# zhuker/lamejs

Measured on NVIDIA H100. Metric: encoded audio seconds/sec (44.1kHz stereo 128kbps CBR), higher is better.
Workload: dtype f64

## Files before the change

lamejs_b200/csrc/k_quant.cuh:

```cuda
#ifndef MP3B200_K_QUANT_CUH
#define MP3B200_K_QUANT_CUH
#include <stddef.h>
#include "mp3_device.cuh"
#include "mp3_tables.h"
#include "k_psy.cuh"

#define Q_LARGE_BITS 100000
#define Q_IXMAX 8206
#define Q_FULL 0xffffffffu

struct GranuleInfoDev {
  int global_gain, part2_3_length, part2_length, big_values, count1, scalefac_compress;
  int table_select[3], region0_count, region1_count, preflag, scalefac_scale, count1table_select, block_type;
  int subblock_gain[4];
  int count1bits, sfbmax, sfbdivide, sfb_lmax, psymax, psy_lmax, sfb_smin, max_nonzero_coeff;
  int scalefac[MP3_SFBMAX];
  int slen[4];
  int part_row;
  int pad_;
  double xrpow_max;
};
struct QuantFrameState {
  int stream, rel_frame;
  int in_old[2], in_step[2];
// ... 9 lines not shown
#define Q_R1S(ch) (4 << (ch))
#define Q_R1(ch) (16 << (ch))
#define Q_R0_ANY 3
#define Q_R1_ANY 48
#define Q_R1S_ANY 12
struct GcPrep { float xmin[MP3_SFBMAX]; int have, mnz, block_type; double xrpow_max; };

__device__ unsigned short g_huff_code[1666];
__device__ unsigned char g_huff_len[1666];
__constant__ int c_huff_off[34];
__constant__ int c_huff_xlen[34];
__device__ int g_t32l[16];
__device__ int g_t33l[16];
__constant__ int c_slen1_n[16];
__constant__ int c_slen2_n[16];
__device__ int g_slen_n[2][16];
__device__ int g_scale_tab[2][16];
__device__ unsigned int g_cat_tab[8][256];
__constant__ int c_slen1_tab[16];
__constant__ int c_slen2_tab[16];
__constant__ int c_huf_noesc[15];

static int quant_upload_constants() {
  static const int t32l[16] = {1, 5, 5, 7, 5, 8, 7, 9, 5, 7, 7, 9, 7, 9, 9, 10};
  static const int t33l[16] = {4, 5, 5, 6, 5, 6, 6, 7, 5, 6, 6, 7, 6, 7, 7, 8};
  static const int s1n[16] = {1, 1, 1, 1, 8, 2, 2, 2, 4, 4, 4, 8, 8, 8, 16, 16};
  static const int s2n[16] = {1, 2, 4, 8, 1, 2, 4, 8, 2, 4, 8, 2, 4, 8, 4, 8};
  static const int s1t[16] = {0, 0, 0, 0, 3, 1, 1, 1, 2, 2, 2, 3, 3, 3, 4, 4};
  static const int s2t[16] = {0, 1, 2, 3, 0, 1, 2, 3, 1, 2, 3, 1, 2, 3, 2, 3};
  static const int ss[16] = {0, 18, 36, 54, 54, 36, 54, 72, 54, 72, 90, 72, 90, 108, 108, 126};
// ... 16 lines not shown
        unsigned a = 0, b = 0, d = 0;
        if (x < xl && y < xl) {
          const int i = x * xl + y;
          if (c == 0) a = b = d = MP3_HUFF_LEN[MP3_HUFF_OFF[1] + i];
          else if (c == 1) { a = MP3_HUFF_TABLE23[i] >> 16; b = d = MP3_HUFF_TABLE23[i] & 0xffff; }
          else if (c == 2) { a = MP3_HUFF_TABLE56[i] >> 16; b = d = MP3_HUFF_TABLE56[i] & 0xffff; }
          else { a = MP3_HUFF_LEN[MP3_HUFF_OFF[t1] + i]; b = MP3_HUFF_LEN[MP3_HUFF_OFF[t1 + 1] + i]; d = MP3_HUFF_LEN[MP3_HUFF_OFF[t1 + 2] + i]; }
        }
        ct[c][q] = a | (b << 11) | (d << 22);
      }
      { const unsigned a = MP3_HUFF_LARGETBL[q] >> 16, b = MP3_HUFF_LARGETBL[q] & 0xffff; ct[6][q] = a | (b << 11) | (b << 22); }
      ct[7][q] = 0;
    }
    UP(g_slen_n, sn); UP(g_scale_tab, st); UP(g_cat_tab, ct);
  }
#undef UP
  return 0;
}

struct __align__(16) GcWork {
  float xrpow[576];
  short ixw[576];
  short* ixg;
  GranuleInfoDev w, b;
  const Mp3Geo* geo;
  float xmin[MP3_SFBMAX], distort[MP3_SFBMAX];
  int pn_step[MP3_SFBMAX]; float pn_noise[MP3_SFBMAX], pn_noise_log[MP3_SFBMAX];
  int pn_global_gain, pn_sfb_count1;
  unsigned char mode[MP3_SFBMAX + 1];
  short nstart[MP3_SFBMAX], nlen[MP3_SFBMAX];
// ... 4 lines not shown
struct __align__(16) WarpShared {
  double ath[6];
  int scfsi[4];
  GcWork wk;
};
#define Q_STRIDE_NOXR ((int)((offsetof(WarpShared, wk) + offsetof(GcWork, xr) + 15) & ~(size_t)15))
static_assert((offsetof(WarpShared, wk) + offsetof(GcWork, xr)) % 16 == 0 && (offsetof(WarpShared, wk) + offsetof(GcWork, xrpow)) % 16 == 0 &&
              (offsetof(WarpShared, wk) + offsetof(GcWork, ixw)) % 16 == 0 && sizeof(WarpShared) % 16 == 0, "rows are moved as 16-byte vectors");
#ifndef Q_SLIM_BLOCKS
#define Q_SLIM_BLOCKS 9
#endif

#define LANE (threadIdx.x & 31)
#ifdef Q_TASKSTAT
__device__ int g_taskstat[1 << 16][8];
#endif
#ifdef Q_STATS
__device__ unsigned long long g_qstats[16];
#define QSTAT(i) do { if (LANE == 0) atomicAdd(&g_qstats[i], 1ull); } while (0)
#else
#define QSTAT(i) do { } while (0)
#endif
#define Q_PRAGMA(x) _Pragma(#x)
#define Q_UNROLL(n) Q_PRAGMA(unroll n)
#ifndef Q_RT_UNROLL
#define Q_RT_UNROLL 1
#endif
#ifndef Q_CB_UNROLL
#define Q_CB_UNROLL 1
#endif
// ... 82 lines not shown
#ifdef MP3_DOMAIN_CHECK
  {
    unsigned fa = 0, fb = 0, fc = 0;
    for (int p = p0; p < p1; p += 32) {
      const unsigned v = rc.cat == 6 ? pair_bits(w32[p], 6, rc.lin) : __ldg(&g_cat_tab[rc.cat][((w32[p] & 0xfu) << 4) | (w32[p] >> 16)]);
      fa += v & 0x7ffu; fb += (v >> 11) & 0x7ffu; fc += v >> 22;
    }
    DOMAIN_MISS(DOM_BITSUM_FIELD, fa > 0x7ffu || fb > 0x7ffu || fc > 0x3ffu || wsumu(fa) > 0xffffu || wsumu(fb) > 0xffffu);
  }
#endif
  const unsigned ab = wsumu((s & 0x7ffu) | (((s >> 11) & 0x7ffu) << 16));
  const int c = wsum((int)(s >> 22));
  return region_pick(mx, rc, (int)(ab & 0xffffu), (int)(ab >> 16), c, bits);
}

__device__ __forceinline__ int noquant_count_bits_w(const Mp3Tables* T, const short* ix, GranuleInfoDev* gi, GcWork* wk, bool use_prev, int top) {
  const int lane = LANE;
  const unsigned* w32 = reinterpret_cast<const unsigned*>(ix);
  const int count1 = wmax(top);
  int a1 = 0, a2 = 0, nq = 0;
  const int qmax = count1 >> 2;
  bool stop = false;
#pragma unroll 1
  for (int q0 = 0; q0 < qmax && !stop; q0 += 32) {
    const int q = q0 + lane;
    int bad = 1, v1 = 0, v2 = 0;
    if (q < qmax) {
      const int i = count1 - 4 * q;
      const unsigned wa = w32[(i - 4) >> 1], wb = w32[(i - 2) >> 1];
      if (((wa | wb) & 0xfffefffeu) == 0) {
        bad = 0;
        const int p = (int)(((wa & 1u) << 3) | ((wa >> 16) << 2) | ((wb & 1u) << 1) | (wb >> 16));
        v1 = __ldg(&g_t32l[p]); v2 = __ldg(&g_t33l[p]);
      }
    }
    const unsigned m = __ballot_sync(Q_FULL, bad);
    const int first_bad = m ? __ffs(m) - 1 : 32;
    if (lane >= first_bad) { v1 = 0; v2 = 0; }
    a1 += wsum(v1); a2 += wsum(v2);
    nq += first_bad;
    if (first_bad < 32) stop = true;
  }
  if (nq > qmax) nq = qmax;
  const int bigv = count1 - 4 * nq;
  int bits = a1, c1sel = 0;
  if (a1 > a2) { bits = a2; c1sel = 1; }
  const int count1bits = bits;
  int r0 = gi->region0_count, r1 = gi->region1_count;
  int ts0 = gi->table_select[0], ts1 = gi->table_select[1], ts2 = gi->table_select[2];
  if (bigv != 0) {
    int b1, b2;
    const int bt = gi->block_type;
    if (bt == BT_SHORT) {
      b1 = 3 * T->sfb_s[3];
      b2 = bigv;
    } else if (bt == BT_NORM) {
      b1 = r0 = T->bv_scf[bigv - 2];
      b2 = r1 = T->bv_scf[bigv - 1];
      b2 = T->sfb_l[b1 + b2 + 2];
      b1 = T->sfb_l[b1 + 1];
    } else {
      r0 = 7; r1 = 22 - 1 - 7 - 1;
      b1 = T->sfb_l[7 + 1];
      b2 = bigv;
    }
    b1 = min(b1, bigv);
    b2 = min(b2, bigv);
    if (bt == BT_NORM && b2 < bigv) { QSTAT(15); ts2 = region_table_w(ix, b2, bigv, &bits); }
    if (0 < b1) { QSTAT(15); ts0 = region_table_w(ix, 0, b1, &bits); }
    if (b1 < b2) { QSTAT(15); ts1 = region_table_w(ix, b1, b2, &bits); }
  }
  __syncwarp();
  if (lane == 0) {
    gi->count1 = count1; gi->count1table_select = c1sel; gi->count1bits = count1bits; gi->big_values = bigv;
    gi->region0_count = r0; gi->region1_count = r1;
    gi->table_select[0] = ts0; gi->table_select[1] = ts1; gi->table_select[2] = ts2;
    if (use_prev) {
      int sc = 0;
      if (bigv != 0 && gi->block_type == BT_NORM) {
        if (bigv >= 576) sc = 22;
        else { sc = T->geo[0].sfb_of_line[bigv]; if (T->sfb_l[sc] != bigv) sc++; }
      }
      wk->pn_sfb_count1 = sc;
    }
  }
  __syncwarp();
  return bits;
}

__device__ __forceinline__ int pretab_of(int sfb) { return sfb < 22 ? (int)((0x2fe95400000ull >> (2 * sfb)) & 3ull) : 0; }

__device__ __forceinline__ int sfb_step(const GranuleInfoDev* gi, const GcWork* wk, int sfb) {
  return gi->global_gain - ((gi->scalefac[sfb] + (gi->preflag != 0 ? pretab_of(sfb) : 0)) << (gi->scalefac_scale + 1)) -
         gi->subblock_gain[wk->geo->window[sfb]] * 8;
}

template <bool use_prev>
__device__ __forceinline__ int count_bits_w(const Mp3Tables* T, GcWork* wk, GranuleInfoDev* gi, short* ix) {
  const int lane = LANE;
  const double istep = (double)T->ipow20[gi->global_gain];
  if (gi->xrpow_max > T->ixmax_over_istep[gi->global_gain]) return Q_LARGE_BITS;
  const int sfbmax = gi->block_type == BT_SHORT ? 38 : 21;
  const int mnz = gi->max_nonzero_coeff;
  unsigned* iw32 = reinterpret_cast<unsigned*>(ix);
  const int i0h = min(576, ((mnz + 2) >> 1) << 1) >> 1;
  if (!use_prev) {
    const int qend = (mnz + 1) & ~1;
    int top = 0;
Q_UNROLL(Q_CB_UNROLL)
    for (int p = lane; p < 288; p += 32) {
      unsigned v = 0;
      if (2 * p < qend) {
        const float2 xp = *reinterpret_cast<const float2*>(&wk->xrpow[2 * p]);
        double x0 = (double)xp.x * istep, x1 = (double)xp.y * istep;
        x0 += (double)__ldg(&T->adj43[js_trunc<DOM_TRUNC_QUANT>(x0)]);
        x1 += (double)__ldg(&T->adj43[js_trunc<DOM_TRUNC_QUANT>(x1)]);
// ... 23 lines not shown
      }
      wk->mode[sfb] = (unsigned char)md;
      wk->nstart[sfb] = jst;
    }
    const unsigned m = __ballot_sync(Q_FULL, trunc_here);
    if (m && term == sfbmax + 1) term = s0 + __ffs(m) - 1;
  }
  __syncwarp();
  int zero_from = 576;
  if (term <= sfbmax) {
    const int term_len = mnz - wk->nstart[term] + 1;
    zero_from = term_len > 0 ? ((term_len & 1) ? mnz : mnz + 1) : mnz;
    if (lane == 0) wk->mode[term] = 1;
  }
  __syncwarp();
  const double compare01 = T->cmp01_over_istep[gi->global_gain];
  int top = 0;
Q_UNROLL(Q_CB_UNROLL)
  for (int p = lane; p < 288; p += 32) {
    const int i = 2 * p;
    unsigned v;
    if (i >= zero_from) { v = 0; iw32[p] = 0; }
    else {
      const int md = wk->mode[wk->geo->sfb_of_line[i]];
      const bool z1 = (i + 1) >= zero_from;
      if (md == 0) {
        v = iw32[p];
        if (z1) { v &= 0xffffu; iw32[p] = v; }
      } else {
        const float2 xp = *reinterpret_cast<const float2*>(&wk->xrpow[i]);
        unsigned v0, v1;
        if (md == 2) { v0 = (compare01 > (double)xp.x) ? 0u : 1u; v1 = (compare01 > (double)xp.y) ? 0u : 1u; }
        else {
          double x0 = (double)xp.x * istep, x1 = (double)xp.y * istep;
          x0 += (double)__ldg(&T->adj43[js_trunc<DOM_TRUNC_QUANT>(x0)]);
          x1 += (double)__ldg(&T->adj43[js_trunc<DOM_TRUNC_QUANT>(x1)]);
          v0 = (unsigned)js_trunc<DOM_TRUNC_QUANT>(x0); v1 = (unsigned)js_trunc<DOM_TRUNC_QUANT>(x1);
          DOMAIN_MISS(DOM_PACK_OUTER, x0 >= 32768.0 || x1 >= 32768.0);
        }
        if (z1) v1 = 0;
        v = v0 | (v1 << 16);
        iw32[p] = v;
      }
    }
    if (v != 0 && p < i0h) top = 2 * p + 2;
  }
  __syncwarp();
  return noquant_count_bits_w(T, ix, gi, wk, use_prev, top);
}

struct NoiseRes { int over_count; double over_SSD, max_noise; int bits; };
__device__ __forceinline__ void calc_noise_w(const Mp3Tables* T, GcWork* wk, const GranuleInfoDev* gi, const short* ix, NoiseRes* res) {
  const int lane = LANE;
  const int psymax = gi->psymax, mnz = gi->max_nonzero_coeff;
  int first_trunc = psymax;
#pragma unroll 1
  for (int s0 = 0; s0 < psymax; s0 += 32) {
    const int sfb = s0 + lane;
    int crosses = 0;
    if (sfb < psymax) {
      const int j = wk->geo->start[sfb], w = wk->geo->width[sfb];
      if (wk->pn_step[sfb] == sfb_step(gi, wk, sfb)) wk->nlen[sfb] = -1;
      else { wk->nstart[sfb] = (short)j; wk->nlen[sfb] = (short)(w >> 1); crosses = (j + w) > mnz; }
    }
    const unsigned m = __ballot_sync(Q_FULL, crosses);
    if (m && first_trunc == psymax) first_trunc = s0 + __ffs(m) - 1;
  }
  __syncwarp();
  if (lane == 0 && first_trunc < psymax) {
    int j = wk->geo->start[first_trunc];
#pragma unroll 1
    for (int sfb = first_trunc; sfb < psymax; sfb++) {
      const int w = wk->geo->width[sfb];
      if (wk->nlen[sfb] < 0) { j += w; continue; }
      int l = w >> 1;
      if ((j + w) > mnz) { const int us = mnz - j + 1; l = us > 0 ? us >> 1 : 0; }
      wk->nstart[sfb] = (short)j; wk->nlen[sfb] = (short)l;
      j += 2 * l;
    }
  }
  __syncwarp();
  int over = 0, ssd = 0; double mxn = -20.0;
#pragma unroll 1
  for (int s0 = 0; s0 < psymax; s0 += 32) {
    const int sfb = s0 + lane;
    if (sfb < psymax) {
      const int s = sfb_step(gi, wk, sfb);
      const bool cached = wk->nlen[sfb] < 0;
      double noise;
      if (cached) noise = (double)wk->pn_noise[sfb];
      else {
        const double step = (double)T->pow20[s + MP3_QMAX2];
        int j = wk->nstart[sfb];
        noise = 0;
Q_UNROLL(Q_CN_UNROLL)
        for (int l = wk->nlen[sfb]; l > 0; l--, j += 2) {
          const float2 x = *reinterpret_cast<const float2*>(&wk->xr[j]);
          const unsigned q0 = reinterpret_cast<const unsigned short*>(ix)[j], q1 = reinterpret_cast<const unsigned short*>(ix)[j + 1];
          double temp;
          temp = fabs((double)x.x) - (double)__ldg(&T->pow43[q0]) * step; noise += temp * temp;
          temp = fabs((double)x.y) - (double)__ldg(&T->pow43[q1]) * step; noise += temp * temp;
        }
        wk->pn_step[sfb] = s;
        { f32s t; t = noise; wk->pn_noise[sfb] = t.v; }
      }
      noise = noise / (double)wk->xmin[sfb];
      { f32s t; t = noise; wk->distort[sfb] = t.v; }
      if (cached) noise = (double)wk->pn_noise_log[sfb];
      else {
        noise = q_log10(js_dmax(noise, 1E-20));
        { f32s t; t = noise; wk->pn_noise_log[sfb] = t.v; }
      }
      if (noise > 0.0) {
        int tmp = js_trunc<DOM_TRUNC_NOISE>(noise * 10 + .5);
        if (tmp < 1) tmp = 1;
        ssd += tmp * tmp;
        over++;
      }
      mxn = js_dmax(mxn, noise);
    }
  }
#pragma unroll 1
  for (int o = 16; o > 0; o >>= 1) {
    const double other = __shfl_xor_sync(Q_FULL, mxn, o);
    mxn = js_dmax(mxn, other);
  }
  over = wsum(over);
  if (lane == 0) wk->pn_global_gain = gi->global_gain;
  __syncwarp();
  res->over_count = over; res->over_SSD = (double)wsum(ssd); res->max_noise = mxn;
}

__device__ __forceinline__ bool scale_bitcount_w(GranuleInfoDev* gi) {
  const int lane = LANE;
  int* scalefac = gi->scalefac;
  const bool is_short = gi->block_type == BT_SHORT;
  const int sfbmax = gi->sfbmax, sfbdivide = gi->sfbdivide;
  __syncwarp();
  if (!is_short && 0 == gi->preflag) {
    const bool in = lane >= 11 && lane < 21;
    const int pt = pretab_of(lane);
    const bool ok = !in || scalefac[lane] >= pt;
    if (__all_sync(Q_FULL, ok)) {
      __syncwarp();
      if (in) scalefac[lane] -= pt;
// ... 45 lines not shown
  return mode_gr == 2 ? scale_bitcount_w(gi) : scale_bitcount_lsf_w(gi);
}

__device__ __forceinline__ bool loop_break_w(const GranuleInfoDev* gi, const GcWork* wk) {
  bool nz = true;
#pragma unroll 1
  for (int sfb = LANE; sfb < gi->sfbmax; sfb += 32)
    if (gi->scalefac[sfb] + gi->subblock_gain[wk->geo->window[sfb]] == 0) nz = false;
  return __all_sync(Q_FULL, nz);
}

__device__ __forceinline__ void scale_xrpow_w(GcWork* wk, GranuleInfoDev* gi, double f34) {
  const int lane = LANE;
  const int sfbmax = gi->sfbmax;
  float mx = 0.0f;
#pragma unroll 1
  for (int p = lane; p < 288; p += 32) {
    const int sfb = wk->geo->sfb_of_line[2 * p];
    if (sfb < sfbmax && wk->mode[sfb]) {
      float2* xp = reinterpret_cast<float2*>(&wk->xrpow[2 * p]);
      float2 x = *xp;
      f32s v0, v1; v0.v = x.x; v1.v = x.y;
      v0 *= f34; v1 *= f34;
      x.x = v0.v; x.y = v1.v;
      *xp = x;
      mx = fmaxf(mx, fmaxf(v0.v, v1.v));
    }
  }
#pragma unroll 1
  for (int o = 16; o > 0; o >>= 1) mx = fmaxf(mx, __shfl_xor_sync(Q_FULL, mx, o));
  if (lane == 0 && (double)mx > gi->xrpow_max) gi->xrpow_max = (double)mx;
  __syncwarp();
}
// ... 89 lines not shown
    const int sfbmax = gi->sfbmax;
    double trigger = 0;
#pragma unroll 1
    for (int sfb = lane; sfb < sfbmax; sfb += 32) if (trigger < (double)wk->distort[sfb]) trigger = (double)wk->distort[sfb];
    for (int o = 16; o > 0; o >>= 1) { const double t = __shfl_xor_sync(Q_FULL, trigger, o); if (trigger < t) trigger = t; }
    if (trigger > 1.0) trigger = sqrt(trigger);
    else trigger *= .95;
#pragma unroll 1
    for (int sfb = lane; sfb < sfbmax; sfb += 32) {
      const int amp = !((double)wk->distort[sfb] < trigger);
      wk->mode[sfb] = (unsigned char)amp;
      if (amp) gi->scalefac[sfb]++;
    }
  }
  __syncwarp();
  scale_xrpow_w(wk, gi, ifq);
  int r;
  if (loop_break_w(gi, wk)) r = 0;
  else r = scale_bitcount_any_w(gi, T->mode_gr) ? 2 : 1;
  if (r == 0) return false;
  if (r == 1) return true;
  return balance_escalate_w(T, wk);
}

__device__ __forceinline__ void copy_gi_w(GranuleInfoDev* dst, const GranuleInfoDev* src) {
  const int n = sizeof(GranuleInfoDev) / 4;
  const int* s = reinterpret_cast<const int*>(src);
  int* d = reinterpret_cast<int*>(dst);
  __syncwarp();
  static_assert(sizeof(GranuleInfoDev) / 4 <= 96, "three rounds");
  int v[3];
#pragma unroll
  for (int k = 0; k < 3; k++) { const int i = LANE + 32 * k; if (i < n) v[k] = s[i]; }
#pragma unroll
  for (int k = 0; k < 3; k++) { const int i = LANE + 32 * k; if (i < n) d[i] = v[k]; }
  __syncwarp();
}
// ... 54 lines not shown

__device__ __forceinline__ unsigned long long gi_hash(const GranuleInfoDev* gi) {
  const unsigned* w = reinterpret_cast<const unsigned*>(gi);
  unsigned sum = 0, x = 0;
#pragma unroll 1
  for (int i = LANE; i < (int)(sizeof(GranuleInfoDev) / 4); i += 32) {
    unsigned v = (w[i] ^ ((unsigned)i * 0x9E3779B9u)) * 0x85EBCA6Bu;
    v ^= v >> 13; v *= 0xC2B2AE35u; v ^= v >> 16;
    sum += v; x ^= __funnelshift_l(v, v, i & 31);
  }
  sum = __reduce_add_sync(Q_FULL, sum);
  x = __reduce_xor_sync(Q_FULL, x);
  return ((unsigned long long)sum << 32) | x;
}

__device__ __forceinline__ void outer_loop_w(const Mp3Tables* T, GcWork* wk, int targ_bits) {
  const int lane = LANE;
  NoiseRes best, cur;
  int best_part2_3_length = 9999999;
#pragma unroll 1
  for (int i = lane; i < MP3_SFBMAX; i += 32) { wk->pn_step[i] = 0; wk->pn_noise[i] = 0.0f; wk->pn_noise_log[i] = 0.0f; }
  if (lane == 0) { wk->pn_global_gain = 0; wk->pn_sfb_count1 = 0; }
  __syncwarp();
  calc_noise_w(T, wk, &wk->b, wk->ixw, &best);
  best.bits = wk->b.part2_3_length;
  copy_gi_w(&wk->w, &wk->b);
  bool best_here = true;
  int age = 0;
  const int quant_comp = T->quant_comp;
  (void)quant_comp;
  do {
    const int search_limit = 3;
    int maxggain = 255;
    if (!balance_noise_w(T, wk)) break;
    GranuleInfoDev* w = &wk->w;
    if (w->scalefac_scale != 0) maxggain = 254;
    const int huff_bits = targ_bits - w->part2_length;
    if (huff_bits <= 0) break;
    int p23, gg;
    if (best_here) { copy_ix_w(wk->ixg, wk->ixw); best_here = false; }
    int sc_in;
    for (;;) {
      sc_in = wk->pn_sfb_count1;
      QSTAT(8);
      p23 = count_bits_w<true>(T, wk, w, wk->ixw);
      gg = w->global_gain;
      __syncwarp();
      if (!(p23 > huff_bits && gg <= maxggain)) break;
      if (lane == 0) w->global_gain = gg + 1;
      __syncwarp();
    }
    if (lane == 0) w->part2_3_length = p23;
    __syncwarp();
    if (gg > maxggain) break;
    if (best.over_count == 0) {
      bool repeat = wk->pn_sfb_count1 == sc_in;
      for (;;) {
        if (!repeat) { QSTAT(9); p23 = count_bits_w<true>(T, wk, w, wk->ixw); }
        repeat = false;
        gg = w->global_gain;
        __syncwarp();
        if (!(p23 > best_part2_3_length && gg <= maxggain)) break;
        if (lane == 0) w->global_gain = gg + 1;
        __syncwarp();
      }
      if (lane == 0) w->part2_3_length = p23;
      __syncwarp();
      if (gg > maxggain) break;
    }
    QSTAT(10);
    calc_noise_w(T, wk, w, wk->ixw, &cur);
    cur.bits = w->part2_3_length;
    bool better;
    if (best.over_count > 0) {
      better = cur.over_SSD <= best.over_SSD;
      if (cur.over_SSD == best.over_SSD) better = cur.bits < best.bits;
    } else {
      better = ((cur.max_noise < 0) && ((cur.max_noise * 10 + cur.bits) <= (best.max_noise * 10 + best.bits)));
    }
    if (best.over_count == 0) better = better && cur.bits < best.bits;
    if (better) {
      best_part2_3_length = wk->b.part2_3_length;
      best = cur;
      copy_gi_w(&wk->b, &wk->w);
      best_here = true;
      age = 0;
    } else {
      if (++age > search_limit && best.over_count == 0) break;
    }
    const int cont = (wk->w.global_gain + wk->w.scalefac_scale) < 255;
    __syncwarp();
    if (!cont) break;
  } while (true);
  if (!best_here) copy_ix_w(wk->ixw, wk->ixg);
}

__device__ __noinline__ double ath_adjust_dev(double a, double x, double athFloor) {
  const double o = 90.30873362, p = 94.82444863;
  double u = q_log10(x) * 10.0;
  const double v = a * a;
  double w = 0.0;
  u -= athFloor;
  if (v > 1E-20) w = 1. + q_log10(v) * (10.0 / o);
  if (w < 0) w = 0.;
  u *= w;
  u += athFloor + o - p;
  return q_pow(10., 0.1 * u);
}

// ... 655 lines not shown
  if (t > 4095) t = 4095;
  int targ = (int)t;
  const int bits = targ * nch;
  if (bits > 7680) { targ = targ * 7680; targ = (int)((double)targ / bits); }
  (void)ch;
  return targ;
}

#ifndef Q_WARPS
#define Q_WARPS 4
#endif
#ifndef Q_BLOCKS_PER_SM
#define Q_BLOCKS_PER_SM 7
#endif
#define Q_THREADS (32 * Q_WARPS)

__device__ __forceinline__ int next_task(int* counter) {
  int t = 0;
  if (LANE == 0) t = atomicAdd(counter, 1);
  return __shfl_sync(Q_FULL, t, 0);
}
template <int STRIDE = (int)sizeof(WarpShared)>
__device__ __forceinline__ WarpShared* warp_shared() {
  extern __shared__ __align__(16) unsigned char smem_raw[];
  return reinterpret_cast<WarpShared*>(smem_raw + (threadIdx.x >> 5) * STRIDE);
}
__device__ __forceinline__ void gi_init_w(GranuleInfoDev* gi, const GcPrep* __restrict__ pr) {
  __syncwarp();
  int* w = reinterpret_cast<int*>(gi);
#pragma unroll 1
// ... 84 lines not shown
  for (int t = next_task(counter); t < ntasks; t = next_task(counter)) {
    const int wi = t / nch, ch = t - wi * nch;
    const int frow = list ? list[wi] : wi;
    QuantFrameState* q = qs + frow;
    const int flags = revalidate ? q->redo : 0;
    if (revalidate == 3 && (flags & Q_R0_ANY)) continue;
    if (revalidate && gr == 1 && !(flags & (Q_R0_ANY | Q_R1S(ch)))) continue;
    const FrameGeom fg = frame_geom(T, streams, q);
    const StreamDesc& sd = streams[fg.z];
    const size_t urow = (size_t)sd.unit_base + T->mode_gr * fg.f + gr, gidx = urow * nch + ch;
    const int targ = granule_budget(nch, fg.mean_bits, gr, q->used0[0], q->used0[1], ch);
    int ov = gr == 0 ? q->in_old[ch] : q->bs_gain0[ch];
    int cs = gr == 0 ? q->in_step[ch] : q->bs_step0[ch];
    const GcPrep* pr = prep + gidx;
    const bool have = pr->have != 0;
    gi_init_w(&wk->b, pr);
    if (lane == 0) wk->geo = &T->geo[pr->block_type == BT_SHORT ? 1 : 0];
    unsigned long long h = 0;
    if (have) {
      copy_row16_w(wk->xrpow, xrpow_g + gidx * 576, 2304);
      QSTAT(revalidate ? 12 + gr : 11);
      bin_search_w(T, wk, targ, &ov, &cs, revalidate ? 2 + 2 * gr : 0);
      h = gi_hash(&wk->b);
    } else {
      __syncwarp();
#pragma unroll 1
      for (int i = lane; i < 288; i += 32) reinterpret_cast<unsigned*>(wk->ixw)[i] = 0;
      __syncwarp();
    }
    bool store;
// ... 25 lines not shown
        q->out_step[ch] = cs;
        if (store) { q->out_old[ch] = ov; q->bs_hash[1][ch] = h; atomicOr(&q->redo, Q_R1(ch)); }
      }
    }
    if (store) {
      copy_row16_w(l3enc + gidx * 576, wk->ixw, 1152);
      copy_gi_w(&ginfo[gidx], &wk->b);
    }
  }
}

__global__ void __launch_bounds__(Q_THREADS, Q_BLOCKS_PER_SM)
k_q_outer(const Mp3Tables* __restrict__ T, const StreamDesc* __restrict__ streams, QuantFrameState* __restrict__ qs,
          GranuleInfoDev* __restrict__ ginfo, short* __restrict__ l3enc, const float* __restrict__ xrq,
          const float* __restrict__ xrpow_g, const GcPrep* __restrict__ prep, int gr, const int* __restrict__ list,
          const int* __restrict__ count_ptr, int count_direct, int revalidate, int* __restrict__ counter) {
  WarpShared* ws = warp_shared();
  GcWork* wk = &ws->wk;
  const int lane = LANE, nch = T->nch;
  const int ntasks = (count_ptr ? *count_ptr : count_direct) * nch;
#pragma unroll 1
  for (int t = next_task(counter); t < ntasks; t = next_task(counter)) {
    const int wi = t / nch, ch = t - wi * nch;
#ifdef Q_REVERSE
    const int frow = list ? list[wi] : (ntasks / nch - 1 - wi);
#else
    const int frow = list ? list[wi] : wi;
#endif
    QuantFrameState* q = qs + frow;
    if (revalidate == 1 && !(q->redo & (gr == 0 ? Q_R0(ch) : Q_R1(ch)))) continue;
    if (revalidate == -1 && (q->redo & Q_R0_ANY)) continue;
    if (revalidate > 0) QSTAT(14);
    const FrameGeom fg = frame_geom(T, streams, q);
    const StreamDesc& sd = streams[fg.z];
    const size_t urow = (size_t)sd.unit_base + T->mode_gr * fg.f + gr, gidx = urow * nch + ch;
    const int targ = granule_budget(nch, fg.mean_bits, gr, q->used0[0], q->used0[1], ch);
    const GcPrep* pr = prep + gidx;
    const bool have = pr->have != 0;
    short* const ixrow = l3enc + gidx * 576;
    __syncwarp();
    if (lane == 0) { wk->geo = &T->geo[pr->block_type == BT_SHORT ? 1 : 0]; wk->ixg = ixrow; }
    copy_gi_w(&wk->b, &ginfo[gidx]);
    copy_row16_w(wk->ixw, ixrow, 1152);
#ifdef Q_TASKSTAT
    const long long ts_t0 = clock64();
    const int ts_gain = wk->b.global_gain, ts_bits = wk->b.part2_3_length;
#endif
    if (have) {
      copy_row16_w(wk->xr, xrq + gidx * 576, 2304);
      copy_row16_w(wk->xrpow, xrpow_g + gidx * 576, 2304);
#pragma unroll 1
      for (int i = lane; i < MP3_SFBMAX; i += 32) wk->xmin[i] = pr->xmin[i];
      __syncwarp();
      outer_loop_w(T, wk, targ);
    }
#ifdef Q_TASKSTAT
    if (lane == 0 && revalidate <= 0 && gidx < (1u << 16)) {
      int* r = g_taskstat[gidx];
      r[0] = (int)((clock64() - ts_t0) >> 6); r[1] = gr; r[2] = wk->b.max_nonzero_coeff; r[3] = wk->b.block_type;
      r[4] = ts_gain; r[5] = ts_bits; r[6] = targ; r[7] = wk->b.global_gain;
    }
#endif
    copy_gi_w(&ginfo[gidx], &wk->b);
    copy_row16_w(ixrow, wk->ixw, 1152);
  }
}

__global__ void __launch_bounds__(Q_THREADS, Q_SLIM_BLOCKS)
k_q_finish(const Mp3Tables* __restrict__ T, const StreamDesc* __restrict__ streams, QuantFrameState* __restrict__ qs,
           GranuleInfoDev* __restrict__ ginfo, short* __restrict__ l3enc, int gr, const int* __restrict__ list,
           const int* __restrict__ count_ptr, int count_direct, int revalidate, int* __restrict__ counter) {
  WarpShared* ws = warp_shared<Q_STRIDE_NOXR>();
  GcWork* wk = &ws->wk;
  const int lane = LANE, nch = T->nch;
  const int ntasks = (count_ptr ? *count_ptr : count_direct) * nch;
#pragma unroll 1
  for (int t = next_task(counter); t < ntasks; t = next_task(counter)) {
    const int wi = t / nch, ch = t - wi * nch;
    const int frow = list ? list[wi] : wi;
// ... 156 lines not shown
  cudaStream_t capture = nullptr;
  int* st = nullptr;
  cudaGraphExec_t exec = nullptr;
};

static int quant_run(const Mp3Tables* dT, const Mp3Tables& hT, StreamDesc* d_streams, int S, int nstreams_with_frames, int max_frames, long long F,
                     const QuantBuffers& B, cudaStream_t st_main, cudaStream_t st_repair, cudaEvent_t ev_fork, cudaEvent_t ev_join,
                     cudaEvent_t ev_pass1, cudaEvent_t* evq, int* evq_pred, int* passes_out, std::atomic<long long>* launches,
                     QuantLoop* dloop = nullptr) {
  cudaStream_t st = st_main;
  static std::mutex attr_mu;
  static bool attr_done[64] = {};
  int dev = 0, sms = 132;
  cudaGetDevice(&dev);
  cudaDeviceGetAttribute(&sms, cudaDevAttrMultiProcessorCount, dev);
  const size_t smem = sizeof(WarpShared) * Q_WARPS, smem_slim = (size_t)Q_STRIDE_NOXR * Q_WARPS, smem_pack = sizeof(PackShared) * Q_WARPS;
  {
    std::lock_guard<std::mutex> lk(attr_mu);
    if (dev < 64 && !attr_done[dev]) {
      if (cudaFuncSetAttribute(k_q_prepare, cudaFuncAttributeMaxDynamicSharedMemorySize, (int)smem) != cudaSuccess) return -100;
      if (cudaFuncSetAttribute(k_q_search, cudaFuncAttributeMaxDynamicSharedMemorySize, (int)smem_slim) != cudaSuccess) return -100;
      if (cudaFuncSetAttribute(k_q_outer, cudaFuncAttributeMaxDynamicSharedMemorySize, (int)smem) != cudaSuccess) return -100;
      if (cudaFuncSetAttribute(k_q_finish, cudaFuncAttributeMaxDynamicSharedMemorySize, (int)smem_slim) != cudaSuccess) return -100;
      if (cudaFuncSetAttribute(k_q_pack, cudaFuncAttributeMaxDynamicSharedMemorySize, (int)smem_pack) != cudaSuccess) return -100;
      attr_done[dev] = true;
    }
  }
  if (F <= 0) { *passes_out = 0; return 0; }
  const int nch = hT.nch;
  int next_counter = Q_NCOUNTERS;
// ... 22 lines not shown
  (*launches)++;
  int* const list1 = B.list;
  int* const list2 = B.list + (F + 1);
  int* const list3 = B.list + 2 * (F + 1);
  auto search = [&](int gr, const int* list, const int* cptr, long long count, int reval) {
    k_q_search<<<grid_for(count * nch, Q_SLIM_BLOCKS), Q_THREADS, smem_slim, st>>>(dT, d_streams, B.qs, B.ginfo, B.l3enc, B.xrpow, B.prep, gr, list, cptr, (int)count,
                                                                             reval, fresh_counter(), list2, B.counter + 1, list3, B.counter + 2);
    (*launches)++;
  };
  int reserve_blocks = 0;
  auto finish = [&](int gr, const int* list, const int* cptr, long long count, int reval) {
    k_q_finish<<<max(1, grid_for(count * nch, Q_SLIM_BLOCKS) - reserve_blocks), Q_THREADS, smem_slim, st>>>(dT, d_streams, B.qs, B.ginfo, B.l3enc, gr, list, cptr, (int)count, reval, fresh_counter());
    (*launches)++;
  };
  auto outer = [&](int gr, const int* list, const int* cptr, long long count, int reval) {
    k_q_outer<<<max(1, grid_for(count * nch, Q_BLOCKS_PER_SM) - reserve_blocks), Q_THREADS, smem, st>>>(dT, d_streams, B.qs, B.ginfo, B.l3enc, B.xrq, B.xrpow, B.prep, gr, list, cptr, (int)count,
                                                                            reval, fresh_counter());
    (*launches)++;
  };
  auto outer_finish = [&](int gr, long long count, int reval, int slot_o, int slot_f) {
    outer(gr, nullptr, nullptr, count, reval); mark(slot_o);
    finish(gr, nullptr, nullptr, count, reval); mark(slot_f);
  };
  auto pack = [&](const int* list, const int* cptr, long long count, int reval) {
    k_q_pack<<<grid_for(count, 9), Q_THREADS, smem_pack, st>>>(dT, d_streams, B.qs, B.ginfo, B.l3enc, B.neg, list, cptr, (int)count, reval, fresh_counter(), nullptr, B.over_budget);
    (*launches)++;
  };
  auto verify = [&](int predict_step = 0) {
    cudaMemsetAsync(B.counter, 0, 3 * sizeof(int), st);
    k_qstate_verify<<<(int)((F + 255) / 256), 256, 0, st>>>(d_streams, B.qs, F, list1, B.counter, predict_step);
    (*launches)++;
  };
// ... 4 lines not shown
    outer_finish(0, F, 0, QE_O0, QE_F0);
    search(1, nullptr, nullptr, F, 0); mark(QE_S1);
  }
  bool forked = false;
  if (Q_SPEC_FOLD && speculated) {
    verify(G == 1 ? 1 : 0);
    search(0, list1, B.counter, F, 1);
    if (G == 2) {
      search(1, list2, B.counter + 1, F, 3);
      int* const c0 = fresh_counter(); int* const c1 = fresh_counter(); int* const c2 = fresh_counter();
      int* const c3 = fresh_counter(); int* const c4 = fresh_counter();
      cudaEventRecord(ev_fork, st_main);
      cudaStreamWaitEvent(st_repair, ev_fork, 0);
      const int gq = Q_REPAIR_BLOCKS, gs = Q_REPAIR_BLOCKS;
      const int* cp = B.counter + 2;
      k_q_outer<<<gq, Q_THREADS, smem, st_repair>>>(dT, d_streams, B.qs, B.ginfo, B.l3enc, B.xrq, B.xrpow, B.prep, 0, list3, cp, (int)F, 1, c0);
      k_q_finish<<<gs, Q_THREADS, smem_slim, st_repair>>>(dT, d_streams, B.qs, B.ginfo, B.l3enc, 0, list3, cp, (int)F, 1, c1);
      k_q_search<<<gs, Q_THREADS, smem_slim, st_repair>>>(dT, d_streams, B.qs, B.ginfo, B.l3enc, B.xrpow, B.prep, 1, list3, cp, (int)F, 1, c2, list2, B.counter + 1,
                                                          list3, B.counter + 2);
      k_q_outer<<<gq, Q_THREADS, smem, st_repair>>>(dT, d_streams, B.qs, B.ginfo, B.l3enc, B.xrq, B.xrpow, B.prep, 1, list3, cp, (int)F, 2, c3);
      k_q_finish<<<gs, Q_THREADS, smem_slim, st_repair>>>(dT, d_streams, B.qs, B.ginfo, B.l3enc, 1, list3, cp, (int)F, 2, c4);
      cudaEventRecord(ev_join, st_repair);
      (*launches) += 5;
      forked = true;
    }
  }
  mark(QE_MID);
  if (G == 2) {
    reserve_blocks = forked ? Q_REPAIR_BLOCKS : 0;
    outer_finish(1, F, forked ? -1 : 0, QE_O1, QE_F1);
    reserve_blocks = 0;
    if (forked) cudaStreamWaitEvent(st_main, ev_join, 0);
  } else {
    outer_finish(0, F, 0, QE_O0, QE_F0);
  }
// ... 70 lines not shown
```

lamejs_b200/csrc/mp3_encoder.cu:

```cuda
#include <cuda_runtime.h>
#include <math.h>
#include <stdio.h>
#include <algorithm>
#include <array>
#include <stdlib.h>
#include <string.h>
#include <atomic>
#include <map>
#include <mutex>
#include <string>
#include <tuple>
#include <vector>

#include "../../include/mp3b200.h"
#include "mp3_config.h"
#include "mp3_device.cuh"
#include "mp3_tables.h"
#include "k_filterbank.cuh"
#include "k_psy.cuh"
#include "k_quant.cuh"
#include "k_tag.cuh"
#include "k_resample.cuh"
#include "k_replaygain.cuh"
#include "k_stage.cuh"
// ... 1880 lines not shown
}

}

#include "mp3_session.inc"
#include "mp3_handle.inc"
#include "mp3_session_handles.inc"

#ifdef Q_TASKSTAT
extern "C" int mp3b200_debug_taskstat(int* out, int rows) {
  if (rows > (1 << 16)) rows = 1 << 16;
  return cudaMemcpyFromSymbol(out, g_taskstat, sizeof(int) * 8 * (size_t)rows) == cudaSuccess ? 0 : -1;
}
#endif

#ifdef PSY_PHASESTAT
extern "C" int mp3b200_debug_psystat(long long* out, int rows) {
  if (rows > PSY_STAT_ROWS) rows = PSY_STAT_ROWS;
  return cudaMemcpyFromSymbol(out, g_psystat, sizeof(long long) * PSY_STAT_COLS * (size_t)rows) == cudaSuccess ? rows : -1;
}
#endif

#ifdef MP3_DOMAIN_CHECK
extern "C" int mp3b200_debug_domain_hits(unsigned long long* out, int cap) {
  if (cap < DOM_NSITES) return DOM_NSITES;
  if (cudaDeviceSynchronize() != cudaSuccess) return -1;
  if (cudaMemcpyFromSymbol(out, g_domain_hits, sizeof(unsigned long long) * DOM_NSITES) != cudaSuccess) return -1;
  static const unsigned long long zero[DOM_NSITES] = {};
  return cudaMemcpyToSymbol(g_domain_hits, zero, sizeof zero) == cudaSuccess ? DOM_NSITES : -1;
}
// ... 2 lines not shown
```

Before: 60760.

## Fuse region table scans, add double pow43/adj43 tables, add phase profiling

Adds a single-pass three-region Huffman table selection for the inner-loop bit counting, so the ix row is scanned once instead of once per region. Precomputes double-precision pow43/adj43 tables in global memory, which removes float-to-double conversions in quantize and noise loops, and uses a cheaper magic-number truncation. Also loads sfb_of_line through the read-only cache and adds compile-time-gated phase-timing instrumentation. The trade is extra device memory and a per-device table upload; region selection is now two passes with branchy per-element region dispatch.

Measured after the change: 62930, median of 6. 3.6% higher.

```diff
diff --git a/lamejs_b200/csrc/k_quant.cuh b/lamejs_b200/csrc/k_quant.cuh
--- a/lamejs_b200/csrc/k_quant.cuh
+++ b/lamejs_b200/csrc/k_quant.cuh
@@ -47,6 +47,8 @@
 __device__ int g_t33l[16];
 __constant__ int c_slen1_n[16];
 __constant__ int c_slen2_n[16];
+#define Q_ADJ43D MP3_PRECALC
+static double* g_q43d[64];
 __device__ int g_slen_n[2][16];
 __device__ int g_scale_tab[2][16];
 __device__ unsigned int g_cat_tab[8][256];
@@ -93,6 +95,18 @@
     }
     UP(g_slen_n, sn); UP(g_scale_tab, st); UP(g_cat_tab, ct);
   }
+  {
+    static Mp3Tables t;
+    static Mp3Resample rs;
+    static Mp3TagParams tag;
+    static double w[2 * MP3_PRECALC];
+    int d = 0;
+    if (cudaGetDevice(&d) != cudaSuccess || d < 0 || d >= 64) return -100;
+    if (mp3_build_config(2, 44100, 128, 0, &t, &rs, &tag) != 0) return -100;
+    for (int i = 0; i < MP3_PRECALC; i++) { w[i] = (double)t.pow43[i]; w[Q_ADJ43D + i] = (double)t.adj43[i]; }
+    if (!g_q43d[d] && cudaMalloc(&g_q43d[d], sizeof w) != cudaSuccess) return -100;
+    if (cudaMemcpy(g_q43d[d], w, sizeof w, cudaMemcpyHostToDevice) != cudaSuccess) return -100;
+  }
 #undef UP
   return 0;
 }
@@ -127,6 +141,42 @@
 #define LANE (threadIdx.x & 31)
 #ifdef Q_TASKSTAT
 __device__ int g_taskstat[1 << 16][8];
+#endif
+#ifdef Q_PHASESTAT
+enum { QP_PRO, QP_CN_WALK, QP_CN_BANDS, QP_CN_RED, QP_BN_AMP, QP_BN_SCALE, QP_BN_BREAK, QP_BN_SBC, QP_CB_MODE, QP_CB_SWEEP,
+       QP_NQ_C1, QP_NQ_REG, QP_COPY, QP_LOOP, QP_EPI, QP_N };
+#define QP_ROWS (1 << 16)
+__device__ unsigned long long g_qphase[QP_ROWS][QP_N][2];
+__device__ long long g_qpslot[256 * 64][2];
+__device__ __forceinline__ long long* qp_slot() {
+  unsigned sm, wid;
+  asm volatile("mov.u32 %0, %%smid;" : "=r"(sm));
+  asm volatile("mov.u32 %0, %%warpid;" : "=r"(wid));
+  return g_qpslot[(sm & 255) * 64 + (wid & 63)];
+}
+__device__ __forceinline__ void qp_begin(long long row) {
+  if (LANE == 0) { long long* s = qp_slot(); s[0] = row; s[1] = clock64(); }
+  __syncwarp();
+}
+__device__ __forceinline__ void qp_mark(int ph) {
+  __syncwarp();
+  if (LANE == 0) {
+    const long long now = clock64();
+    long long* s = qp_slot();
+    const long long row = *(volatile long long*)&s[0];
+    if (row >= 0) {
+      atomicAdd(&g_qphase[row][ph][0], (unsigned long long)(now - *(volatile long long*)&s[1]));
+      atomicAdd(&g_qphase[row][ph][1], 1ull);
+      *(volatile long long*)&s[1] = clock64();
+    }
+  }
+  __syncwarp();
+}
+#define QP_BEGIN(row) qp_begin(row)
+#define QP_MARK(ph) qp_mark(ph)
+#else
+#define QP_BEGIN(row) do { } while (0)
+#define QP_MARK(ph) do { } while (0)
 #endif
 #ifdef Q_STATS
 __device__ unsigned long long g_qstats[16];
@@ -239,6 +289,53 @@
   return region_pick(mx, rc, (int)(ab & 0xffffu), (int)(ab >> 16), c, bits);
 }
 
+__device__ __forceinline__ void region_tables3_w(const short* ix, int b1, int b2, int b3, int* ts0, int* ts1, int* ts2, int* bits) {
+  const int lane = LANE;
+  const unsigned* w32 = reinterpret_cast<const unsigned*>(ix);
+  const int e1 = b1 >> 1, e2 = b2 >> 1, e3 = b3 >> 1;
+  unsigned m0 = 0, m1 = 0, m2 = 0;
+Q_UNROLL(Q_RT_UNROLL)
+  for (int p = lane; p < e3; p += 32) {
+    const unsigned w = w32[p];
+    if (p < e1) m0 = __vmaxu2(m0, w); else if (p < e2) m1 = __vmaxu2(m1, w); else m2 = __vmaxu2(m2, w);
+  }
+  const int mx0 = (int)__reduce_max_sync(Q_FULL, max(m0 & 0xffffu, m0 >> 16));
+  const int mx1 = (int)__reduce_max_sync(Q_FULL, max(m1 & 0xffffu, m1 >> 16));
+  const int mx2 = (int)__reduce_max_sync(Q_FULL, max(m2 & 0xffffu, m2 >> 16));
+  unsigned s0 = 0, s1 = 0, s2 = 0;
+  {
+    const RegionClass rc0 = region_class(mx0), rc1 = region_class(mx1), rc2 = region_class(mx2);
+    const unsigned k0 = rc0.lin | ((unsigned)rc0.cat << 29), k1 = rc1.lin | ((unsigned)rc1.cat << 29), k2 = rc2.lin | ((unsigned)rc2.cat << 29);
+Q_UNROLL(Q_RT_UNROLL)
+    for (int p = lane; p < e3; p += 32) {
+      const bool in0 = p < e1, in1 = !in0 && p < e2;
+      const unsigned k = in0 ? k0 : (in1 ? k1 : k2);
+      const unsigned v = pair_bits(w32[p], (int)(k >> 29), k & 0x1fffffffu);
+      if (in0) s0 += v; else if (in1) s1 += v; else s2 += v;
+    }
+  }
+#ifdef MP3_DOMAIN_CHECK
+  {
+    unsigned f[3][3] = {};
+    for (int p = lane; p < e3; p += 32) {
+      const int r = p < e1 ? 0 : (p < e2 ? 1 : 2);
+      const RegionClass rc = region_class(r == 0 ? mx0 : (r == 1 ? mx1 : mx2));
+      const unsigned v = pair_bits(w32[p], rc.cat, rc.lin);
+      f[r][0] += v & 0x7ffu; f[r][1] += (v >> 11) & 0x7ffu; f[r][2] += v >> 22;
+    }
+    for (int r = 0; r < 3; r++)
+      DOMAIN_MISS(DOM_BITSUM_FIELD, f[r][0] > 0x7ffu || f[r][1] > 0x7ffu || f[r][2] > 0x3ffu || wsumu(f[r][0]) > 0xffffu || wsumu(f[r][1]) > 0xffffu);
+  }
+#endif
+  const unsigned ab0 = wsumu((s0 & 0x7ffu) | (((s0 >> 11) & 0x7ffu) << 16));
+  const unsigned ab1 = wsumu((s1 & 0x7ffu) | (((s1 >> 11) & 0x7ffu) << 16));
+  const unsigned ab2 = wsumu((s2 & 0x7ffu) | (((s2 >> 11) & 0x7ffu) << 16));
+  const int c0 = wsum((int)(s0 >> 22)), c1 = wsum((int)(s1 >> 22)), c2 = wsum((int)(s2 >> 22));
+  if (b2 < b3) { QSTAT(15); *ts2 = region_pick(mx2, region_class(mx2), (int)(ab2 & 0xffffu), (int)(ab2 >> 16), c2, bits); }
+  if (0 < b1) { QSTAT(15); *ts0 = region_pick(mx0, region_class(mx0), (int)(ab0 & 0xffffu), (int)(ab0 >> 16), c0, bits); }
+  if (b1 < b2) { QSTAT(15); *ts1 = region_pick(mx1, region_class(mx1), (int)(ab1 & 0xffffu), (int)(ab1 >> 16), c1, bits); }
+}
+
 __device__ __forceinline__ int noquant_count_bits_w(const Mp3Tables* T, const short* ix, GranuleInfoDev* gi, GcWork* wk, bool use_prev, int top) {
   const int lane = LANE;
   const unsigned* w32 = reinterpret_cast<const unsigned*>(ix);
@@ -267,6 +364,7 @@
     if (first_bad < 32) stop = true;
   }
   if (nq > qmax) nq = qmax;
+  QP_MARK(QP_NQ_C1);
   const int bigv = count1 - 4 * nq;
   int bits = a1, c1sel = 0;
   if (a1 > a2) { bits = a2; c1sel = 1; }
@@ -291,9 +389,13 @@
     }
     b1 = min(b1, bigv);
     b2 = min(b2, bigv);
-    if (bt == BT_NORM && b2 < bigv) { QSTAT(15); ts2 = region_table_w(ix, b2, bigv, &bits); }
-    if (0 < b1) { QSTAT(15); ts0 = region_table_w(ix, 0, b1, &bits); }
-    if (b1 < b2) { QSTAT(15); ts1 = region_table_w(ix, b1, b2, &bits); }
+    if (use_prev) {
+      region_tables3_w(ix, b1, b2, bigv, &ts0, &ts1, &ts2, &bits);
+    } else {
+      if (bt == BT_NORM && b2 < bigv) { QSTAT(15); ts2 = region_table_w(ix, b2, bigv, &bits); }
+      if (0 < b1) { QSTAT(15); ts0 = region_table_w(ix, 0, b1, &bits); }
+      if (b1 < b2) { QSTAT(15); ts1 = region_table_w(ix, b1, b2, &bits); }
+    }
   }
   __syncwarp();
   if (lane == 0) {
@@ -310,7 +412,13 @@
     }
   }
   __syncwarp();
+  QP_MARK(QP_NQ_REG);
   return bits;
+}
+
+__device__ __forceinline__ int q_trunc_nonneg(double x) {
+  DOMAIN_MISS(DOM_TRUNC_QUANT, !(x >= 0.0) || x >= 2147483648.0);
+  return __double2loint(__dadd_rz(x, 6755399441055744.0));
 }
 
 __device__ __forceinline__ int pretab_of(int sfb) { return sfb < 22 ? (int)((0x2fe95400000ull >> (2 * sfb)) & 3ull) : 0; }
@@ -321,10 +429,10 @@
 }
 
 template <bool use_prev>
-__device__ __forceinline__ int count_bits_w(const Mp3Tables* T, GcWork* wk, GranuleInfoDev* gi, short* ix) {
+__device__ __forceinline__ int count_bits_w(const Mp3Tables* T, GcWork* wk, GranuleInfoDev* gi, short* ix, const double* q43d = nullptr) {
   const int lane = LANE;
   const double istep = (double)T->ipow20[gi->global_gain];
-  if (gi->xrpow_max > T->ixmax_over_istep[gi->global_gain]) return Q_LARGE_BITS;
+  if (gi->xrpow_max > T->ixmax_over_istep[gi->global_gain]) { if (use_prev) QP_MARK(QP_CB_MODE); return Q_LARGE_BITS; }
   const int sfbmax = gi->block_type == BT_SHORT ? 38 : 21;
   const int mnz = gi->max_nonzero_coeff;
   unsigned* iw32 = reinterpret_cast<unsigned*>(ix);
@@ -378,7 +486,9 @@
     if (lane == 0) wk->mode[term] = 1;
   }
   __syncwarp();
+  QP_MARK(QP_CB_MODE);
   const double compare01 = T->cmp01_over_istep[gi->global_gain];
+  const unsigned char* const sfb_of_line = wk->geo->sfb_of_line;
   int top = 0;
 Q_UNROLL(Q_CB_UNROLL)
   for (int p = lane; p < 288; p += 32) {
@@ -386,7 +496,7 @@
     unsigned v;
     if (i >= zero_from) { v = 0; iw32[p] = 0; }
     else {
-      const int md = wk->mode[wk->geo->sfb_of_line[i]];
+      const int md = wk->mode[__ldg(&sfb_of_line[i])];
       const bool z1 = (i + 1) >= zero_from;
       if (md == 0) {
         v = iw32[p];
@@ -397,9 +507,9 @@
         if (md == 2) { v0 = (compare01 > (double)xp.x) ? 0u : 1u; v1 = (compare01 > (double)xp.y) ? 0u : 1u; }
         else {
           double x0 = (double)xp.x * istep, x1 = (double)xp.y * istep;
-          x0 += (double)__ldg(&T->adj43[js_trunc<DOM_TRUNC_QUANT>(x0)]);
-          x1 += (double)__ldg(&T->adj43[js_trunc<DOM_TRUNC_QUANT>(x1)]);
-          v0 = (unsigned)js_trunc<DOM_TRUNC_QUANT>(x0); v1 = (unsigned)js_trunc<DOM_TRUNC_QUANT>(x1);
+          x0 += __ldg(&q43d[Q_ADJ43D + q_trunc_nonneg(x0)]);
+          x1 += __ldg(&q43d[Q_ADJ43D + q_trunc_nonneg(x1)]);
+          v0 = (unsigned)q_trunc_nonneg(x0); v1 = (unsigned)q_trunc_nonneg(x1);
           DOMAIN_MISS(DOM_PACK_OUTER, x0 >= 32768.0 || x1 >= 32768.0);
         }
         if (z1) v1 = 0;
@@ -410,11 +520,13 @@
     if (v != 0 && p < i0h) top = 2 * p + 2;
   }
   __syncwarp();
+  QP_MARK(QP_CB_SWEEP);
   return noquant_count_bits_w(T, ix, gi, wk, use_prev, top);
 }
 
 struct NoiseRes { int over_count; double over_SSD, max_noise; int bits; };
-__device__ __forceinline__ void calc_noise_w(const Mp3Tables* T, GcWork* wk, const GranuleInfoDev* gi, const short* ix, NoiseRes* res) {
+__device__ __forceinline__ void calc_noise_w(const Mp3Tables* T, const double* q43d, GcWork* wk, const GranuleInfoDev* gi, const short* ix,
+                                             NoiseRes* res) {
   const int lane = LANE;
   const int psymax = gi->psymax, mnz = gi->max_nonzero_coeff;
   int first_trunc = psymax;
@@ -444,6 +556,7 @@
     }
   }
   __syncwarp();
+  QP_MARK(QP_CN_WALK);
   int over = 0, ssd = 0; double mxn = -20.0;
 #pragma unroll 1
   for (int s0 = 0; s0 < psymax; s0 += 32) {
@@ -462,8 +575,8 @@
           const float2 x = *reinterpret_cast<const float2*>(&wk->xr[j]);
           const unsigned q0 = reinterpret_cast<const unsigned short*>(ix)[j], q1 = reinterpret_cast<const unsigned short*>(ix)[j + 1];
           double temp;
-          temp = fabs((double)x.x) - (double)__ldg(&T->pow43[q0]) * step; noise += temp * temp;
-          temp = fabs((double)x.y) - (double)__ldg(&T->pow43[q1]) * step; noise += temp * temp;
+          temp = fabs((double)x.x) - __ldg(&q43d[q0]) * step; noise += temp * temp;
+          temp = fabs((double)x.y) - __ldg(&q43d[q1]) * step; noise += temp * temp;
         }
         wk->pn_step[sfb] = s;
         { f32s t; t = noise; wk->pn_noise[sfb] = t.v; }
@@ -484,6 +597,7 @@
       mxn = js_dmax(mxn, noise);
     }
   }
+  QP_MARK(QP_CN_BANDS);
 #pragma unroll 1
   for (int o = 16; o > 0; o >>= 1) {
     const double other = __shfl_xor_sync(Q_FULL, mxn, o);
@@ -493,6 +607,7 @@
   if (lane == 0) wk->pn_global_gain = gi->global_gain;
   __syncwarp();
   res->over_count = over; res->over_SSD = (double)wsum(ssd); res->max_noise = mxn;
+  QP_MARK(QP_CN_RED);
 }
 
 __device__ __forceinline__ bool scale_bitcount_w(GranuleInfoDev* gi) {
@@ -568,9 +683,10 @@
   const int lane = LANE;
   const int sfbmax = gi->sfbmax;
   float mx = 0.0f;
+  const unsigned char* const sfb_of_line = wk->geo->sfb_of_line;
 #pragma unroll 1
   for (int p = lane; p < 288; p += 32) {
-    const int sfb = wk->geo->sfb_of_line[2 * p];
+    const int sfb = __ldg(&sfb_of_line[2 * p]);
     if (sfb < sfbmax && wk->mode[sfb]) {
       float2* xp = reinterpret_cast<float2*>(&wk->xrpow[2 * p]);
       float2 x = *xp;
@@ -690,13 +806,19 @@
     }
   }
   __syncwarp();
+  QP_MARK(QP_BN_AMP);
   scale_xrpow_w(wk, gi, ifq);
+  QP_MARK(QP_BN_SCALE);
   int r;
-  if (loop_break_w(gi, wk)) r = 0;
+  const bool brk = loop_break_w(gi, wk);
+  QP_MARK(QP_BN_BREAK);
+  if (brk) r = 0;
   else r = scale_bitcount_any_w(gi, T->mode_gr) ? 2 : 1;
   if (r == 0) return false;
-  if (r == 1) return true;
-  return balance_escalate_w(T, wk);
+  if (r == 1) { QP_MARK(QP_BN_SBC); return true; }
+  const bool ok = balance_escalate_w(T, wk);
+  QP_MARK(QP_BN_SBC);
+  return ok;
 }
 
 __device__ __forceinline__ void copy_gi_w(GranuleInfoDev* dst, const GranuleInfoDev* src) {
@@ -781,7 +903,7 @@
   return ((unsigned long long)sum << 32) | x;
 }
 
-__device__ __forceinline__ void outer_loop_w(const Mp3Tables* T, GcWork* wk, int targ_bits) {
+__device__ __forceinline__ void outer_loop_w(const Mp3Tables* T, const double* q43d, GcWork* wk, int targ_bits) {
   const int lane = LANE;
   NoiseRes best, cur;
   int best_part2_3_length = 9999999;
@@ -789,9 +911,11 @@
   for (int i = lane; i < MP3_SFBMAX; i += 32) { wk->pn_step[i] = 0; wk->pn_noise[i] = 0.0f; wk->pn_noise_log[i] = 0.0f; }
   if (lane == 0) { wk->pn_global_gain = 0; wk->pn_sfb_count1 = 0; }
   __syncwarp();
-  calc_noise_w(T, wk, &wk->b, wk->ixw, &best);
+  QP_MARK(QP_LOOP);
+  calc_noise_w(T, q43d, wk, &wk->b, wk->ixw, &best);
   best.bits = wk->b.part2_3_length;
   copy_gi_w(&wk->w, &wk->b);
+  QP_MARK(QP_COPY);
   bool best_here = true;
   int age = 0;
   const int quant_comp = T->quant_comp;
@@ -799,18 +923,18 @@
   do {
     const int search_limit = 3;
     int maxggain = 255;
-    if (!balance_noise_w(T, wk)) break;
+    if (!balance_noise_w(T, wk)) { QP_MARK(QP_LOOP); break; }
     GranuleInfoDev* w = &wk->w;
     if (w->scalefac_scale != 0) maxggain = 254;
     const int huff_bits = targ_bits - w->part2_length;
     if (huff_bits <= 0) break;
     int p23, gg;
-    if (best_here) { copy_ix_w(wk->ixg, wk->ixw); best_here = false; }
+    if (best_here) { copy_ix_w(wk->ixg, wk->ixw); best_here = false; QP_MARK(QP_COPY); }
     int sc_in;
     for (;;) {
       sc_in = wk->pn_sfb_count1;
       QSTAT(8);
-      p23 = count_bits_w<true>(T, wk, w, wk->ixw);
+      p23 = count_bits_w<true>(T, wk, w, wk->ixw, q43d);
       gg = w->global_gain;
       __syncwarp();
       if (!(p23 > huff_bits && gg <= maxggain)) break;
@@ -823,7 +947,7 @@
     if (best.over_count == 0) {
       bool repeat = wk->pn_sfb_count1 == sc_in;
       for (;;) {
-        if (!repeat) { QSTAT(9); p23 = count_bits_w<true>(T, wk, w, wk->ixw); }
+        if (!repeat) { QSTAT(9); p23 = count_bits_w<true>(T, wk, w, wk->ixw, q43d); }
         repeat = false;
         gg = w->global_gain;
         __syncwarp();
@@ -836,7 +960,8 @@
       if (gg > maxggain) break;
     }
     QSTAT(10);
-    calc_noise_w(T, wk, w, wk->ixw, &cur);
+    QP_MARK(QP_LOOP);
+    calc_noise_w(T, q43d, wk, w, wk->ixw, &cur);
     cur.bits = w->part2_3_length;
     bool better;
     if (best.over_count > 0) {
@@ -852,14 +977,16 @@
       copy_gi_w(&wk->b, &wk->w);
       best_here = true;
       age = 0;
+      QP_MARK(QP_COPY);
     } else {
       if (++age > search_limit && best.over_count == 0) break;
     }
     const int cont = (wk->w.global_gain + wk->w.scalefac_scale) < 255;
     __syncwarp();
+    QP_MARK(QP_LOOP);
     if (!cont) break;
   } while (true);
-  if (!best_here) copy_ix_w(wk->ixw, wk->ixg);
+  if (!best_here) { copy_ix_w(wk->ixw, wk->ixg); QP_MARK(QP_COPY); }
 }
 
 __device__ __noinline__ double ath_adjust_dev(double a, double x, double athFloor) {
@@ -1545,6 +1672,16 @@
 #define Q_BLOCKS_PER_SM 7
 #endif
 #define Q_THREADS (32 * Q_WARPS)
+#ifdef Q_PHASESTAT
+static int q_outer_per_sm() {
+  const char* e = getenv("MP3B200_Q_OUTER_PER_SM");
+  const int n = e ? atoi(e) : 0;
+  return n > 0 && n < Q_BLOCKS_PER_SM ? n : Q_BLOCKS_PER_SM;
+}
+#define Q_OUTER_PER_SM q_outer_per_sm()
+#else
+#define Q_OUTER_PER_SM Q_BLOCKS_PER_SM
+#endif
 
 __device__ __forceinline__ int next_task(int* counter) {
   int t = 0;
@@ -1659,6 +1796,7 @@
     int cs = gr == 0 ? q->in_step[ch] : q->bs_step0[ch];
     const GcPrep* pr = prep + gidx;
     const bool have = pr->have != 0;
+    QP_BEGIN(-1);
     gi_init_w(&wk->b, pr);
     if (lane == 0) wk->geo = &T->geo[pr->block_type == BT_SHORT ? 1 : 0];
     unsigned long long h = 0;
@@ -1714,7 +1852,8 @@
 k_q_outer(const Mp3Tables* __restrict__ T, const StreamDesc* __restrict__ streams, QuantFrameState* __restrict__ qs,
           GranuleInfoDev* __restrict__ ginfo, short* __restrict__ l3enc, const float* __restrict__ xrq,
           const float* __restrict__ xrpow_g, const GcPrep* __restrict__ prep, int gr, const int* __restrict__ list,
-          const int* __restrict__ count_ptr, int count_direct, int revalidate, int* __restrict__ counter) {
+          const int* __restrict__ count_ptr, int count_direct, int revalidate, int* __restrict__ counter,
+          const double* __restrict__ q43d) {
   WarpShared* ws = warp_shared();
   GcWork* wk = &ws->wk;
   const int lane = LANE, nch = T->nch;
@@ -1731,6 +1870,7 @@
     if (revalidate == 1 && !(q->redo & (gr == 0 ? Q_R0(ch) : Q_R1(ch)))) continue;
     if (revalidate == -1 && (q->redo & Q_R0_ANY)) continue;
     if (revalidate > 0) QSTAT(14);
+    QP_BEGIN(revalidate <= 0 ? (long long)((size_t)gr * ntasks + t) % QP_ROWS : -1);
     const FrameGeom fg = frame_geom(T, streams, q);
     const StreamDesc& sd = streams[fg.z];
     const size_t urow = (size_t)sd.unit_base + T->mode_gr * fg.f + gr, gidx = urow * nch + ch;
@@ -1752,7 +1892,8 @@
 #pragma unroll 1
       for (int i = lane; i < MP3_SFBMAX; i += 32) wk->xmin[i] = pr->xmin[i];
       __syncwarp();
-      outer_loop_w(T, wk, targ);
+      QP_MARK(QP_PRO);
+      outer_loop_w(T, q43d, wk, targ);
     }
 #ifdef Q_TASKSTAT
     if (lane == 0 && revalidate <= 0 && gidx < (1u << 16)) {
@@ -1763,6 +1904,7 @@
 #endif
     copy_gi_w(&ginfo[gidx], &wk->b);
     copy_row16_w(ixrow, wk->ixw, 1152);
+    QP_MARK(QP_EPI);
   }
 }
 
@@ -1949,6 +2091,8 @@
   int dev = 0, sms = 132;
   cudaGetDevice(&dev);
   cudaDeviceGetAttribute(&sms, cudaDevAttrMultiProcessorCount, dev);
+  const double* const q43d = dev >= 0 && dev < 64 ? g_q43d[dev] : nullptr;
+  if (!q43d) return -100;
   const size_t smem = sizeof(WarpShared) * Q_WARPS, smem_slim = (size_t)Q_STRIDE_NOXR * Q_WARPS, smem_pack = sizeof(PackShared) * Q_WARPS;
   {
     std::lock_guard<std::mutex> lk(attr_mu);
@@ -2001,8 +2145,8 @@
     (*launches)++;
   };
   auto outer = [&](int gr, const int* list, const int* cptr, long long count, int reval) {
-    k_q_outer<<<max(1, grid_for(count * nch, Q_BLOCKS_PER_SM) - reserve_blocks), Q_THREADS, smem, st>>>(dT, d_streams, B.qs, B.ginfo, B.l3enc, B.xrq, B.xrpow, B.prep, gr, list, cptr, (int)count,
-                                                                            reval, fresh_counter());
+    k_q_outer<<<max(1, grid_for(count * nch, Q_OUTER_PER_SM) - reserve_blocks), Q_THREADS, smem, st>>>(dT, d_streams, B.qs, B.ginfo, B.l3enc, B.xrq, B.xrpow, B.prep, gr, list, cptr, (int)count,
+                                                                            reval, fresh_counter(), q43d);
     (*launches)++;
   };
   auto outer_finish = [&](int gr, long long count, int reval, int slot_o, int slot_f) {
@@ -2037,11 +2181,11 @@
       cudaStreamWaitEvent(st_repair, ev_fork, 0);
       const int gq = Q_REPAIR_BLOCKS, gs = Q_REPAIR_BLOCKS;
       const int* cp = B.counter + 2;
-      k_q_outer<<<gq, Q_THREADS, smem, st_repair>>>(dT, d_streams, B.qs, B.ginfo, B.l3enc, B.xrq, B.xrpow, B.prep, 0, list3, cp, (int)F, 1, c0);
+      k_q_outer<<<gq, Q_THREADS, smem, st_repair>>>(dT, d_streams, B.qs, B.ginfo, B.l3enc, B.xrq, B.xrpow, B.prep, 0, list3, cp, (int)F, 1, c0, q43d);
       k_q_finish<<<gs, Q_THREADS, smem_slim, st_repair>>>(dT, d_streams, B.qs, B.ginfo, B.l3enc, 0, list3, cp, (int)F, 1, c1);
       k_q_search<<<gs, Q_THREADS, smem_slim, st_repair>>>(dT, d_streams, B.qs, B.ginfo, B.l3enc, B.xrpow, B.prep, 1, list3, cp, (int)F, 1, c2, list2, B.counter + 1,
                                                           list3, B.counter + 2);
-      k_q_outer<<<gq, Q_THREADS, smem, st_repair>>>(dT, d_streams, B.qs, B.ginfo, B.l3enc, B.xrq, B.xrpow, B.prep, 1, list3, cp, (int)F, 2, c3);
+      k_q_outer<<<gq, Q_THREADS, smem, st_repair>>>(dT, d_streams, B.qs, B.ginfo, B.l3enc, B.xrq, B.xrpow, B.prep, 1, list3, cp, (int)F, 2, c3, q43d);
       k_q_finish<<<gs, Q_THREADS, smem_slim, st_repair>>>(dT, d_streams, B.qs, B.ginfo, B.l3enc, 1, list3, cp, (int)F, 2, c4);
       cudaEventRecord(ev_join, st_repair);
       (*launches) += 5;
diff --git a/lamejs_b200/csrc/mp3_encoder.cu b/lamejs_b200/csrc/mp3_encoder.cu
--- a/lamejs_b200/csrc/mp3_encoder.cu
+++ b/lamejs_b200/csrc/mp3_encoder.cu
@@ -1918,6 +1918,20 @@
 }
 #endif
 
+#ifdef Q_PHASESTAT
+extern "C" int mp3b200_debug_qphase(unsigned long long* out, int rows, int clear) {
+  if (rows > QP_ROWS) rows = QP_ROWS;
+  if (cudaDeviceSynchronize() != cudaSuccess) return -1;
+  if (out && cudaMemcpyFromSymbol(out, g_qphase, sizeof(unsigned long long) * QP_N * 2 * (size_t)rows) != cudaSuccess) return -1;
+  if (clear) {
+    void* p = nullptr;
+    if (cudaGetSymbolAddress(&p, g_qphase) != cudaSuccess || cudaMemset(p, 0, sizeof(g_qphase)) != cudaSuccess) return -1;
+    if (cudaDeviceSynchronize() != cudaSuccess) return -1;
+  }
+  return QP_N;
+}
+#endif
+
 #ifdef PSY_PHASESTAT
 extern "C" int mp3b200_debug_psystat(long long* out, int rows) {
   if (rows > PSY_STAT_ROWS) rows = PSY_STAT_ROWS;
```
